# geometrian/simple-spectral

Measured on AMD Instinct MI355X. Metric: Msamples/s (w*h*spp/s) cornell-srgb 512x512, higher is better.
Workload: dtype f32

## Files before the change

include/ssx.h:

```cpp
#ifndef SSX_H
#define SSX_H

#include <stddef.h>
#include <stdint.h>

#ifdef __cplusplus
extern "C" {
#endif

#define SSX_ABI_VERSION 2

enum {
	SSX_OK = 0,
	SSX_ERR_DATA = -1,
	SSX_ERR_ARG = -2,
	SSX_ERR_SCENE = -3,
	SSX_ERR_DEVICE = -10,
	SSX_ERR_STATE = -11
};

#define SSX_MAX_DEPTH 10u
#define SSX_TILE_SIZE 8u
#define SSX_SAMPLE_WAVELENGTHS 4u
#define SSX_MAX_TEXTURES 64u
// ... 232 lines not shown

int ssx_delta_e_images(ssx_ctx* ctx, uint32_t width, uint32_t height, const float* xyz_a, const float* xyz_b, const double white_a[3], const double white_b[3],
                       const uint8_t* labels , uint32_t regions, const double t[2], float* de , float* lab ,
                       double* SUM, double* SSQ, float* MAX, uint64_t* NF, uint64_t* NX, uint64_t* EX );
int ssx_spectral_delta_e(ssx_ctx* ctx, const ssx_denoise_params* denoise , int denoised_a, int denoised_b, const float* weights_a ,
                         const float* weights_b , const double white_a[3], const double white_b[3], const uint8_t* labels , uint32_t regions,
                         const double t[2], float* de , float* lab ,
                         double* SUM, double* SSQ, float* MAX, uint64_t* NF, uint64_t* NX, uint64_t* EX );

enum {
	SSX_DBG_FMATH = 1,
	SSX_DBG_SPHTRI = 2,
	SSX_DBG_ARVO = 3,
	SSX_DBG_SAMPLE_LIGHT = 4,
	SSX_DBG_COSHEMI = 5,
	SSX_DBG_TRACE = 6,
	SSX_DBG_RAND_CHOICE = 7,
	SSX_DBG_ALBEDO = 8,
	SSX_DBG_FLUX_TO_XYZ = 9,
	SSX_DBG_RAND_1F = 10,
	SSX_DBG_GLIBC_MATH = 11,
	SSX_DBG_SPHTRI_GLIBC = 12, SSX_DBG_ARVO_GLIBC = 13, SSX_DBG_SAMPLE_LIGHT_GLIBC = 14, SSX_DBG_COSHEMI_GLIBC = 15,
	SSX_DBG_TRACE_MASKED = 16,
	SSX_DBG_TRACE_TOPO = 17
};
enum {
	SSX_SWEEP_RCP = 1,
	SSX_SWEEP_SQRT = 2,
	SSX_SWEEP_INVERSESQRT = 3,
	SSX_SWEEP_SIN = 4,
	SSX_SWEEP_COS = 5,
	SSX_SWEEP_ACOS = 6,
	SSX_SWEEP_DIV_PI = 7,
	SSX_SWEEP_RCP64 = 8,
	SSX_SWEEP_DIV_PAIRS = 9,
	SSX_SWEEP_ACOS_SIN = 10,
	SSX_SWEEP_SIN_PROOF = 11, SSX_SWEEP_COS_PROOF = 12, SSX_SWEEP_ACOS_PROOF = 13,
	SSX_SWEEP_GLIBC_SIN = 14, SSX_SWEEP_GLIBC_COS = 15, SSX_SWEEP_GLIBC_ACOS = 16,
	SSX_SWEEP_GLIBC_COS_LDS = 17
};
int ssx_debug_sweep(ssx_ctx* ctx, uint32_t op, uint32_t lo, uint64_t count, uint64_t result[11]);
int ssx_debug_pass1_source(const uint8_t* vid, uint32_t n_quads, const char* name, char* out, size_t out_size);
int ssx_debug_eval(ssx_ctx* ctx, uint32_t op, const void* in, uint32_t in_words, void* out, uint32_t out_words, uint32_t n);
int ssx_debug_samples(ssx_ctx* ctx, const ssx_render_params* params, float* xyza, uint64_t* rng_state, uint32_t* levels);
int ssx_debug_sample_flux(ssx_ctx* ctx, const ssx_render_params* params, float* flux, float* lambda_0);
int ssx_debug_tile_mask(ssx_ctx* ctx, const ssx_render_params* params, uint32_t* out);
int ssx_debug_spectral_accumulate(ssx_ctx* ctx, uint32_t width, uint32_t height, uint32_t bins, uint32_t tile_first, uint32_t tile_stride, uint32_t tile_skew,
// ... 62 lines not shown
```

simple_spectral_amd/_capi.py:

```python
import ctypes as C
import os

from . import build as _build


class SsxSpectrum(C.Structure):
    _fields_ = [("offset", C.c_uint32), ("n", C.c_uint32), ("low", C.c_float), ("high", C.c_float),
                ("delta_recip", C.c_float)]


class SsxVertex(C.Structure):
    _fields_ = [("pos", C.c_float * 3), ("st", C.c_float * 2)]


class SsxQuad(C.Structure):
    _fields_ = [("v00", SsxVertex), ("v10", SsxVertex), ("v11", SsxVertex), ("v01", SsxVertex),
                ("normal0", C.c_float * 3), ("normal1", C.c_float * 3),
                ("material", C.c_uint32), ("flags", C.c_uint32)]


class SsxMaterial(C.Structure):
    _fields_ = [("kind", C.c_uint32), ("albedo_mode", C.c_uint32), ("albedo_spectrum", C.c_uint32),
                ("albedo_texture", C.c_uint32), ("emission_spectrum", C.c_uint32)]

# ... 88 lines not shown
               "ssx_spectral_import",
               "ssx_set_spectral_moments", "ssx_spectral_variance", "ssx_spectral_probe", "ssx_probe_arrays",
               "ssx_spectral_noise", "ssx_spectral_noise_reduce",
               "ssx_spectral_moments_import",
               "ssx_spectral_compare", "ssx_spectral_compare_arrays",
               "ssx_delta_e_images", "ssx_spectral_delta_e",
               "ssx_debug_tile_mask", "ssx_debug_spectral_accumulate", "ssx_debug_fold", "ssx_debug_step"]
SSX_FOLD_ROW_WORDS, SSX_FOLD_LAMBDA0, SSX_FOLD_CAM_DIR, SSX_FOLD_HIT, SSX_FOLD_N, SSX_FOLD_LEVEL0, SSX_FOLD_LEVEL_WORDS = 160, 0, 1, 4, 5, 10, 15
SSX_FOLD_L_FS, SSX_FOLD_L_NDL, SSX_FOLD_L_PDF, SSX_FOLD_L_FLAGS, SSX_FOLD_L_EMISSION, SSX_FOLD_L_NEE = 0, 4, 5, 6, 7, 11
SSX_FOLD_EMISSION, SSX_FOLD_NEE, SSX_FOLD_NEE_VISIBLE = 1, 2, 4
SSX_STEP_ROW_WORDS, SSX_STEP_R_ORIG, SSX_STEP_R_DIR, SSX_STEP_R_IGNORE, SSX_STEP_R_DEPTH, SSX_STEP_R_LAMBDA0, SSX_STEP_R_RNG, SSX_STEP_R_PREV_SLOT = 16, 0, 3, 6, 7, 8, 9, 13
SSX_STEP_NO_SLOT, SSX_STEP_OUT_WORDS = 0x1FFF, 40
(SSX_STEP_O_FLAGS, SSX_STEP_O_HIT_TRI, SSX_STEP_O_HIT_DIST, SSX_STEP_O_HIT_ST, SSX_STEP_O_EMISSION, SSX_STEP_O_NEE, SSX_STEP_O_NEE_TERM, SSX_STEP_O_FS, SSX_STEP_O_NDL,
 SSX_STEP_O_PDF, SSX_STEP_O_PREV_SLOT, SSX_STEP_O_TAIL_DEPTH, SSX_STEP_O_TAIL_HIT, SSX_STEP_O_NEXT_ORIG, SSX_STEP_O_NEXT_DIR, SSX_STEP_O_NEXT_IGNORE,
 SSX_STEP_O_NEXT_DEPTH, SSX_STEP_O_RNG, SSX_STEP_O_SLOT) = 0, 1, 2, 3, 5, 9, 13, 17, 21, 22, 23, 24, 25, 26, 29, 32, 33, 34, 36
SSX_STEP_HIT, SSX_STEP_CONTINUED, SSX_STEP_EMISSION, SSX_STEP_PARKED, SSX_STEP_VISIBLE = 1, 2, 4, 8, 16
(SSX_SWEEP_RCP, SSX_SWEEP_SQRT, SSX_SWEEP_INVERSESQRT, SSX_SWEEP_SIN, SSX_SWEEP_COS, SSX_SWEEP_ACOS, SSX_SWEEP_DIV_PI,
 SSX_SWEEP_RCP64, SSX_SWEEP_DIV_PAIRS, SSX_SWEEP_ACOS_SIN, SSX_SWEEP_SIN_PROOF, SSX_SWEEP_COS_PROOF, SSX_SWEEP_ACOS_PROOF) = range(1, 14)
(SSX_DBG_FMATH, SSX_DBG_SPHTRI, SSX_DBG_ARVO, SSX_DBG_SAMPLE_LIGHT, SSX_DBG_COSHEMI, SSX_DBG_TRACE, SSX_DBG_RAND_CHOICE,
 SSX_DBG_ALBEDO, SSX_DBG_FLUX_TO_XYZ, SSX_DBG_RAND_1F) = range(1, 11)
(SSX_DBG_GLIBC_MATH, SSX_DBG_SPHTRI_GLIBC, SSX_DBG_ARVO_GLIBC, SSX_DBG_SAMPLE_LIGHT_GLIBC, SSX_DBG_COSHEMI_GLIBC) = range(11, 16)
(SSX_SWEEP_GLIBC_SIN, SSX_SWEEP_GLIBC_COS, SSX_SWEEP_GLIBC_ACOS, SSX_SWEEP_GLIBC_COS_LDS) = range(14, 18)
SSX_DBG_TRACE_TOPO = 17
SSX_DBG_TRACE_MASKED = 16
HOST_SYMBOLS = ["ssh_scene_create", "ssh_scene_create_ex", "ssh_scene_destroy", "ssh_scene_desc", "ssh_xyza_to_srgba", "ssh_save_image",
                "ssh_load_png_rgb8", "ssh_free", "ssh_color_values", "ssh_last_error", "ssh_checkpoint_save", "ssh_checkpoint_load", "ssh_sums_merge", "ssh_save_npy_f32",
                "ssh_develop_weights", "ssh_relight_gain", "ssh_emitter_spectrum",
                "ssh_checkpoint_save_spectral", "ssh_checkpoint_load_spectral", "ssh_spectral_merge",
                "ssh_probe_derive", "ssh_probe_save_csv", "ssh_spectral_noise_derive", "ssh_spectral_noise_save_csv",
                "ssh_checkpoint_save_moments", "ssh_checkpoint_load_moments", "ssh_moments_merge",
                "ssh_compare_derive", "ssh_compare_save_csv",
                "ssh_delta_e_derive", "ssh_delta_e_save_csv", "ssh_develop_white"]

_hip = None
_host = None


def host_lib():
    global _host
    if _host is None:
        path = _build.HOST_LIB
        if not os.path.exists(path):
            _build.build_host()
        lib = C.CDLL(path)
        vp = C.c_void_p
        lib.ssh_last_error.restype = C.c_char_p
# ... 230 lines not shown
```

simple_spectral_amd/csrc/ssx_api.hip:

```cpp
#include "ssx_kernels.hip"
#include "ssx_debug.hip"

#include "../../include/ssx.h"

#include <chrono>
#include <array>
#include <atomic>
#include <cstdarg>
#include <cstdio>
#include <cstdlib>
#include <cmath>
#include <algorithm>
#include <cstring>
#include <mutex>
#include <string>
#include <thread>
#include <vector>

#include <limits.h>
#include <set>

#include "ssx_jit.h"

namespace {
// ... 1066 lines not shown
	SSX_HIP(ctx, hipMemcpy(d_in.ptr, in, (size_t)n * in_words * 4, hipMemcpyHostToDevice));
	SsxKernelArgs a{};
	a.blob = ctx->d_blob.as<uint32_t>(); a.blob_words = ctx->blob_words; a.rgb_mode = ctx->rgb_mode ? 1u : 0u;
	const size_t lds = staged_blob_lds(ctx->blob_words);
	if (op == SSX_DBG_TRACE_MASKED && in_words < 11u) return fail(ctx, SSX_ERR_ARG, "SSX_DBG_TRACE_MASKED: a row is orig[3], dir[3], ignore, mask[4]");
	if (op == SSX_DBG_TRACE_TOPO) {
		if (in_words < 8u) return fail(ctx, SSX_ERR_ARG, "SSX_DBG_TRACE_TOPO: a row is orig[3], dir[3], ignore, has_ray");
		if (ctx->topology == 0u) return fail(ctx, SSX_ERR_STATE, "SSX_DBG_TRACE_TOPO: the context runs the generic trace (topology 0); that is SSX_DBG_TRACE");
		const uint32_t* d_rows = d_in.as<uint32_t>(); uint32_t* d_res = d_out.as<uint32_t>();
		void* args[] = { &a, &d_rows, &in_words, &d_res, &out_words, &n };
		if (ctx->topology == 3u) {
			std::string err;
			const ssx_jit::Kernels* k = ssx_jit::get(ctx->device, ctx->jit_vid, &err, ssx_jit::kVariantDebug);
			if (!k || !k->debug_trace) return fail(ctx, SSX_ERR_STATE, "SSX_DBG_TRACE_TOPO: the debug kernel of the scene's pattern could not be compiled: " + err);
			SSX_HIP(ctx, hipModuleLaunchKernel(k->debug_trace, (n + 255u) / 256u, 1, 1, 256, 1, 1, (unsigned)lds, ctx->stream, args, nullptr));
		} else {
			const void* host = ctx->topology == 1u ? (const void*)ssx_debug_trace_cornell_kernel : (const void*)ssx_debug_trace_plane_kernel;
			SSX_HIP(ctx, hipLaunchKernel(host, dim3((n + 255u) / 256u), dim3(256), args, lds, ctx->stream));
		}
		SSX_HIP(ctx, hipStreamSynchronize(ctx->stream));
		SSX_HIP(ctx, hipMemcpy(out, d_out.ptr, (size_t)n * out_words * 4, hipMemcpyDeviceToHost));
		return SSX_OK;
	}
	const auto kernel =op >= SSX_DBG_GLIBC_MATH && op <= SSX_DBG_COSHEMI_GLIBC ? ssx_debug_eval_glibc_kernel : ssx_debug_eval_kernel;
	hipLaunchKernelGGL(kernel, dim3((n + 255u) / 256u), dim3(256), lds, ctx->stream, a, op, d_in.as<uint32_t>(), in_words, d_out.as<uint32_t>(), out_words, n);
	SSX_HIP(ctx, hipGetLastError());
	SSX_HIP(ctx, hipStreamSynchronize(ctx->stream));
	SSX_HIP(ctx, hipMemcpy(out, d_out.ptr, (size_t)n * out_words * 4, hipMemcpyDeviceToHost));
	return SSX_OK;
}

int ssx_debug_sweep(ssx_ctx* ctx, uint32_t op, uint32_t lo, uint64_t count, uint64_t result[11]) {
	if (!ctx || !result || count == 0 || count > (1ull << 32)) return SSX_ERR_ARG;
	if (!ctx->have_scene) return fail(ctx, SSX_ERR_STATE, "no scene uploaded");
	if (ctx->rendering.load()) return fail(ctx, SSX_ERR_STATE, "render in progress");
	SSX_HIP(ctx, hipSetDevice(ctx->device));
	DeviceBuffer d_res;
	SSX_HIP(ctx, d_res.reserve(11 * sizeof(unsigned long long)));
	SSX_HIP(ctx, hipMemsetAsync(d_res.ptr, 0, 11 * sizeof(unsigned long long), ctx->stream));
	SsxKernelArgs a{};
	a.blob = ctx->d_blob.as<uint32_t>(); a.blob_words = ctx->blob_words;
	const size_t lds = staged_blob_lds(ctx->blob_words);
	const auto kernel = op >= SSX_SWEEP_GLIBC_SIN ? ssx_debug_sweep_glibc_kernel : ssx_debug_sweep_kernel;
	hipLaunchKernelGGL(kernel, dim3(256 * 16), dim3(256), lds, ctx->stream, a, op, lo, (uint64_t)count, d_res.as<unsigned long long>());
	SSX_HIP(ctx, hipGetLastError());
	SSX_HIP(ctx, hipStreamSynchronize(ctx->stream));
// ... 334 lines not shown
```

simple_spectral_amd/csrc/ssx_debug.hip:

```cpp
#include "../../include/ssx.h"
#include "ssx_ddmath.h"

namespace {

__device__ __forceinline__ Rng load_rng(const uint32_t* w) {
	Rng r;
	r.state = ((uint64_t)w[1] << 32) | w[0];
	r.inc = ((uint64_t)w[3] << 32) | w[2];
	return r;
}
__device__ __forceinline__ float f(uint32_t u) { return __uint_as_float(u); }
__device__ __forceinline__ uint32_t u(float x) { return __float_as_uint(x); }

}

__device__ __forceinline__ uint32_t sweep_hash(uint32_t h) {
	h ^= h >> 16; h *= 0x7FEB352Du; h ^= h >> 15; h *= 0x846CA68Bu; h ^= h >> 16;
	return h;
}
__device__ __forceinline__ bool same_float(float a, float b) { return __float_as_uint(a) == __float_as_uint(b) || (a != a && b != b); }
extern "C" __global__ void __launch_bounds__(256) ssx_debug_sweep_kernel(SsxKernelArgs a, uint32_t op, uint32_t lo, uint64_t count, unsigned long long* res) {
	Lds L; L.w = stage_lds(a);
	(void)L;
	unsigned long long bad = 0, mx = 0;
// ... 157 lines not shown
		float xyz[3];
		flux_to_xyz(L, fl, f(x[4]), xyz);
		o[0] = u(xyz[0]); o[1] = u(xyz[1]); o[2] = u(xyz[2]);
		break;
	}
	case SSX_DBG_RAND_1F: {
		Rng r = load_rng(x);
		o[0] = u(rand_1f(r)); o[1] = (uint32_t)r.state; o[2] = (uint32_t)(r.state >> 32);
		break;
	}
	default: break;
	}
	if (gid < n)
		for (uint32_t k = 0; k < out_words && k < 12u; ++k) out[(size_t)gid * out_words + k] = o[k];
}

#define SSX_DEBUG_TRACE_TOPO_KERNEL(name, topo) \
	extern "C" __global__ void __launch_bounds__(256) name(SsxKernelArgs a, const uint32_t* in, uint32_t in_words, uint32_t* out, uint32_t out_words, uint32_t n) { \
		debug_trace_rows<topo>(a, in, in_words, out, out_words, n); \
	}
SSX_DEBUG_TRACE_TOPO_KERNEL(ssx_debug_trace_cornell_kernel, 1)
SSX_DEBUG_TRACE_TOPO_KERNEL(ssx_debug_trace_plane_kernel, 2)
#undef SSX_DEBUG_TRACE_TOPO_KERNEL

__device__ __forceinline__ uint32_t fold_rank(uint32_t rc, uint32_t seed) { return (rc * ((seed << 1) | 1u) + (seed >> 8)) & (SSX_COHORT_RECORDS - 1u); }
template <bool NARROW, bool GLIBC, bool FLUX>
__device__ __forceinline__ void debug_fold_body(const SsxKernelArgs& a, const uint32_t* rows, uint32_t n_tiles, uint32_t n_k, uint32_t order_seed, uint32_t parked) {
	static_assert((SSX_COHORT_RECORDS & (SSX_COHORT_RECORDS - 1u)) == 0u, "fold_rank permutes a power of two");
	uint32_t* const lds_words = stage_lds<GLIBC>(a);
	Lds L; L.w = lds_words;
	const uint32_t wave = threadIdx.x >> 6, lane = threadIdx.x & 63u;
	const uint32_t wave_slot = blockIdx.x * 4u + wave;
	if (wave_slot >= n_tiles) return;
	uint32_t* const cnt = lds_words + a.blob_words + wave * SSX_WAVE_COUNTER_WORDS;
	const uint32_t rec_base = wave_slot * n_k * 64u;
	const uint32_t* const tile_rows = rows + (size_t)wave_slot * 64u * n_k * SSX_FOLD_ROW_WORDS;
	LogRef lg; lg.cnt = cnt; lg.wave_base = wave_slot * 2u * a.unit_cohorts;
	for (uint32_t kq = 0; kq < n_k; kq += SSX_COHORT_KS) {
		const uint32_t cohort = kq / SSX_COHORT_KS, ways = min(SSX_COHORT_KS, n_k - kq);
		for (uint32_t s = 0; s < ways; ++s) {
			const uint32_t rc = s * 64u + lane, my_rank = fold_rank(rc, order_seed);
			uint32_t fs0 = 0, ne0 = 0;
			for (uint32_t o = 0; o < ways * 64u; ++o) {
				if (fold_rank(o, order_seed) >= my_rank) continue;
				const uint32_t* y = tile_rows + ((size_t)(o & 63u) * n_k + kq + (o >> 6)) * SSX_FOLD_ROW_WORDS;
				const uint32_t on = min(y[SSX_FOLD_N], SSX_MAX_FRAMES);
// ... 280 lines not shown
```

simple_spectral_amd/csrc/ssx_jit.h:

```cpp
#pragma once
#include <hip/hip_runtime.h>
#include <dlfcn.h>

#include <sys/stat.h>
#include <unistd.h>

#include <algorithm>
#include <array>
#include <chrono>
#include <condition_variable>
#include <cstdint>
#include <cstdio>
#include <cstdlib>
#include <cstring>
#include <deque>
#include <map>
#include <mutex>
#include <set>
#include <string>
#include <thread>
#include <utility>
#include <vector>

#include "ssx_sources_gen.h"
// ... 88 lines not shown
	int (*log_size)(Program, size_t*) = nullptr;
	int (*log)(Program, char*) = nullptr;
	int (*code_size)(Program, size_t*) = nullptr;
	int (*code)(Program, char*) = nullptr;
	int (*destroy)(Program*) = nullptr;
	bool open(std::string* err) {
		if (lib) return true;
		for (const char* name : { "libhiprtc.so.7", "libhiprtc.so", "/opt/rocm/lib/libhiprtc.so" }) if ((lib = dlopen(name, RTLD_NOW | RTLD_LOCAL))) break;
		if (!lib) { const char* why = dlerror(); *err = std::string("hipRTC is not available (") + (why ? why : "dlopen failed") + ")"; return false; }
		bool ok = true;
		auto sym = [&](const char* n) { void* s = dlsym(lib, n); ok = ok && s; return s; };
		create = (decltype(create))sym("hiprtcCreateProgram"); compile = (decltype(compile))sym("hiprtcCompileProgram");
		log_size = (decltype(log_size))sym("hiprtcGetProgramLogSize"); log = (decltype(log))sym("hiprtcGetProgramLog");
		code_size = (decltype(code_size))sym("hiprtcGetCodeSize"); code = (decltype(code))sym("hiprtcGetCode");
		destroy = (decltype(destroy))sym("hiprtcDestroyProgram");
		if (!ok) { *err = "hipRTC lacks an entry point"; dlclose(lib); lib = nullptr; }
		return ok;
	}
};

struct Kernels {
	hipModule_t module = nullptr;
	hipFunction_t path = nullptr, path_nq = nullptr;
	hipFunction_t debug_trace = nullptr;
};

enum class State { Missing, Pending, Ready, Failed };

inline uint64_t fnv64(const void* data, size_t n, uint64_t h = 0xCBF29CE484222325ull) {
	const unsigned char* p = static_cast<const unsigned char*>(data);
	for (size_t i = 0; i < n; ++i) { h ^= p[i]; h *= 0x100000001B3ull; }
	return h;
}

struct Shared {
	std::mutex m;
	std::condition_variable cv;
	std::map<std::string, std::string> code, errors;
	std::set<std::string> queued;
	std::deque<std::pair<std::string, std::pair<VidTable, uint32_t>>> jobs;
	bool worker_running = false;
	std::map<std::pair<int, std::string>, Kernels> modules;
	std::set<std::string> disk_missed;
	std::mutex rtc_mutex;
	Rtc rtc;
	uint64_t compiled = 0, disk_hits = 0;
};
// ... 115 lines not shown
	if (libm_flag(libm)) opts.push_back(libm_flag(libm));
	const int rc = rtc.compile(prog, (int)opts.size(), opts.data());
	if (rc != 0) {
		size_t n = 0; rtc.log_size(prog, &n);
		std::string log(n, '\0'); if (n) rtc.log(prog, &log[0]);
		*err = "hipRTC could not compile the specialised kernels: " + log.substr(0, 600);
		rtc.destroy(&prog);
		return false;
	}
	size_t n = 0; rtc.code_size(prog, &n);
	obj->resize(n); rtc.code(prog, &(*obj)[0]);
	rtc.destroy(&prog);
	return true;
}

inline const Kernels* load_locked(Shared& S, int device, const std::string& key, std::string* err) {
	auto it = S.modules.find({ device, key });
	if (it != S.modules.end()) return &it->second;
	const std::string& obj = S.code[key];
	Kernels k;
	hipError_t e = hipModuleLoadData(&k.module, obj.data());
	if (key.compare(0, 6, "debug|") == 0) {
		if (e == hipSuccess) e = hipModuleGetFunction(&k.debug_trace, k.module, "ssx_debug_trace_jit");
	} else {
		if (e == hipSuccess) e = hipModuleGetFunction(&k.path, k.module, "ssx_render_kernel_jit");
		if (e == hipSuccess) e = hipModuleGetFunction(&k.path_nq, k.module, "ssx_render_kernel_jit_nq");
	}
	if (e != hipSuccess) {
		*err = std::string("loading the specialised kernels failed: ") + hipGetErrorString(e);
		if (k.module) (void)hipModuleUnload(k.module);
		S.errors[key] = *err; S.code.erase(key);
		return nullptr;
	}
	return &(S.modules[{ device, key }] = k);
}

inline State lookup(int device, const VidTable& vids, const Kernels** out, std::string* err, uint32_t libm = 0) {
	Shared& S = shared();
	const std::string key = pattern_key(vids, libm);
	{
		std::lock_guard<std::mutex> g(S.m);
		auto bad = S.errors.find(key);
		if (bad != S.errors.end()) { *err = bad->second; return State::Failed; }
		if (S.code.count(key)) { *out = load_locked(S, device, key, err); return *out ? State::Ready : State::Failed; }
		if (S.queued.count(key)) return State::Pending;
		if (S.disk_missed.count(key)) return State::Missing;
// ... 75 lines not shown
```

simple_spectral_amd/csrc/ssx_kernels.hip:

```cpp
#include <hip/hip_runtime.h>
#ifndef __HIPCC_RTC__
#include <stdint.h>
#endif

#include "ssx_blob.h"
#include "ssx_exact.h"
#include "ssx_lanestat.h"
extern __shared__ __attribute__((aligned(16))) uint32_t ssx_lds[];
#define SSX_FM_TABLE (reinterpret_cast<const double*>(ssx_lds))
#ifdef SSX_JIT_BUILD
#include "ssx_fmath.h"
#else
#include "../../include/ssx_fmath.h"
#endif
#define SSX_GM_TABLE (SSX_FM_TABLE + SSX_FM_I_A11)
#ifdef SSX_JIT_BUILD
#include "ssx_glibc_math.h"
#else
#include "../../include/ssx_glibc_math.h"
#endif
__device__ const double ssx_fm_coeff_values[SSX_FM_N_COEFF] = SSX_FM_COEFF_INIT;
__device__ const double ssx_gm_coeff_values[SSX_GM_N_COEFF] = SSX_GM_COEFF_INIT;
static_assert(2 * SSX_FM_N_COEFF <= SSX_LDS_PREFIX_WORDS, "coefficient table");
static_assert(SSX_FM_I_A11 + SSX_GM_N_COEFF <= SSX_FM_N_COEFF, "glibc coefficients in the arc-cosine slots");
// ... 505 lines not shown
				double Ud = (double)B.y * (double)C.x - (double)B.x * (double)C.y;
				double Vd = (double)C.y * (double)A.x - (double)C.x * (double)A.y;
				double Wd = (double)A.y * (double)B.x - (double)A.x * (double)B.y;
				if ((Ud < 0.0 || Vd < 0.0 || Wd < 0.0) && (Ud > 0.0 || Vd > 0.0 || Wd > 0.0)) continue;
				U = (float)Ud; V = (float)Vd; W = (float)Wd;
			}
			float det = U + V + W;
			if (!(__builtin_fabsf(det) > SSX_EPS)) continue;
			float Az = rs.Sz * A.z, Bz = rs.Sz * B.z, Cz = rs.Sz * C.z;
			float T = U * Az + V * Bz + W * Cz;
			if ((__float_as_uint(det) ^ __float_as_uint(T)) & 0x80000000u) continue;
			float det_recip = ssx_exact::rcp(det);
			float dist = T * det_recip;
			if (dist >= SSX_EPS && dist < hit.dist) {
				hit.tri = (int)(2u * base + bit); hit.dist = dist;
				hit.U = U; hit.V = V; hit.W = W; hit.det_recip = det_recip;
				if (which == 0u) cand &= ~(1ull << (bit + 1u));
			}
		}
		if (tm) SSX_TIME_AFTER(*tm, stat_base == 0 ? 8 : 13, hit.dist);
	}
}

struct SphTri {
	V3 A, B, C;
	float b, cos_c;
	float alpha, cos_alpha, sin_alpha;
	float area;
};

template <bool GLIBC = false>
__device__ __forceinline__ void sphtri_make_general(V3 A, V3 B, V3 C, SphTri& t) {
	auto acos_ = [](float x) { return GLIBC ? ssx_glibc_acosf(x) : ssx_acosf_lds(x); };
	auto sin_ = [](float x) { return GLIBC ? ssx_glibc_sinf(x) : ssx_sinf_lds(x); };
	const float under_pi = __uint_as_float(0x40490FDAu);
	const float nanv = __uint_as_float(0x7FC00000u);
	float cos_a = clamp_glm(dot3(B, C), -1.0f, 1.0f);
	float cos_b = clamp_glm(dot3(A, C), -1.0f, 1.0f);
	float cos_c = clamp_glm(dot3(A, B), -1.0f, 1.0f);
	float a = clamp_glm(acos_(cos_a), 0.0f, under_pi);
	float b = clamp_glm(acos_(cos_b), 0.0f, under_pi);
	float c = clamp_glm(acos_(cos_c), 0.0f, under_pi);
	float sin_a = sin_(a), sin_b = sin_(b), sin_c = sin_(c);
	float numer0 = cos_a - cos_b * cos_c;
	float numer1 = cos_b - cos_c * cos_a;
	float numer2 = cos_c - cos_a * cos_b;
// ... 269 lines not shown
	float bx = hit.U * hit.det_recip, by = hit.V * hit.det_recip, bz = hit.W * hit.det_recip;
	const float* s0 = Q.st[0];
	const float* s1 = which ? Q.st[2] : Q.st[1];
	const float* s2 = which ? Q.st[3] : Q.st[2];
	st_x = (bx * s0[0] + by * s1[0]) + bz * s2[0];
	st_y = (bx * s0[1] + by * s1[1]) + bz * s2[1];
}

template <int TOPO>
__device__ __forceinline__ void debug_trace_rows(const SsxKernelArgs& a, const uint32_t* in, uint32_t in_words, uint32_t* out, uint32_t out_words, uint32_t n) {
	Lds L; L.w = stage_lds(a);
	const uint32_t gid = blockIdx.x * blockDim.x + threadIdx.x;
	const uint32_t item = gid < n ? gid : n - 1u;
	const uint32_t* x = in + (size_t)item * in_words;
	HitInfo h;
	trace<TOPO>(L, mk(__uint_as_float(x[0]), __uint_as_float(x[1]), __uint_as_float(x[2])), mk(__uint_as_float(x[3]), __uint_as_float(x[4]), __uint_as_float(x[5])),
	            (int)x[6], x[7] != 0u, h);
	uint32_t o[5] = { h.tri < 0 ? 0xFFFFFFFFu : (uint32_t)h.tri >> 1, h.tri < 0 ? 0u : (uint32_t)h.tri & 1u, __float_as_uint(h.dist), 0u, 0u };
	if (h.tri >= 0) { float sx, sy; hit_st(L.quad((uint32_t)h.tri >> 1), (uint32_t)h.tri & 1u, h, sx, sy); o[3] = __float_as_uint(sx); o[4] = __float_as_uint(sy); }
	if (gid < n)
		for (uint32_t k = 0; k < out_words && k < 5u; ++k) out[(size_t)gid * out_words + k] = o[k];
}

template <bool NARROW, bool BLACK, bool GLIBC = false>
__device__ __forceinline__ bool path_step(const Lds& L, const ShadowQ& q, const SsxKernelArgs& a, const LogRef& lg, Path& p, bool& pushed, uint32_t& level_word) {
	const SsxBlobHeader& h = L.hdr();
	level_word = level_word_none();
	SSX_STAT(4);
	const uint32_t hq = (uint32_t)p.hit_tri >> 1, which = (uint32_t)p.hit_tri & 1u;
	const SsxBlobQuad& Q = L.quad(hq);
	const SsxBlobQuad& M = Q;
	V3 N = mk(Q.normal[which][0], Q.normal[which][1], Q.normal[which][2]);

	float direct[4] = { 0.0f, 0.0f, 0.0f, 0.0f };
	const bool els = a.no_els == 0u;
	if ((els ? (p.depth == 0u && !a.indirect_only) : true) && M.is_emissive != 0u) {
		SSX_STAT(5);
		Hero em = spectrum_hero(L, M.emission, p.lambda_0, h.lambda_step);
#pragma unroll
		for (int k = 0; k < 4; ++k) direct[k] += em.v[k];
		store_emission(a, lg, p.depth, p.rec_index, direct);
		level_word = level_word_emission(level_word);
	}
	if (p.depth + 1u >= SSX_MAX_DEPTH_) return false;
	const V3 hit_pos = add(p.orig, scl(p.hit_dist, p.dir));
	p.orig = hit_pos;
// ... 70 lines not shown
	}
	if (!cont || (els && p.depth + 2u >= SSX_MAX_DEPTH_)) return false;
	SSX_STAT(12);
	const uint32_t slot = log_append(lg, 0u);
	store_level_entry(a, lg, slot, f_s, n_dot_l, pdf_w_i, p.prev_slot, level_word);
	wave_release(lg.cnt);
	p.prev_slot = slot;
	p.dir = w_i; p.ignore = (int)hq;
	++p.depth;
	return true;
}

template <int TOPO, bool NARROW>
__device__ __forceinline__ void shadow_flush(const Lds& L, const SsxKernelArgs& a, const ShadowQ& q, uint32_t first, uint32_t n, SsxTimer& tm) {
	const uint32_t lane = threadIdx.x & 63u;
	const bool have = lane < n;
	const bool narrow = NARROW;
	float4 e0 = make_float4(0.0f, 0.0f, 0.0f, 0.0f), e1 = make_float4(0.0f, 1.0f, 0.0f, 0.0f), e2 = e0;
	if (have) {
		if (narrow) { const float4* E = q.e + 2u * (first + lane); e0 = E[0]; e1 = E[1]; e2.z = e1.z; e2.w = e1.w; }
		else { const float4* E = q.e + 3u * (first + lane); e0 = E[0]; e1 = E[1]; e2 = E[2]; }
	}
	const uint32_t tag = __float_as_uint(e2.z);
	HitInfo sh;
	trace<TOPO>(L, mk(e0.x, e0.y, e0.z), mk(e0.w, e1.x, e1.y), (int)(tag & 0xFFu), have, sh, 2, nullptr, &tm);
	if (have) {
		const bool visible = sh.tri >= 0 && ((uint32_t)sh.tri >> 1) == (tag >> 8);
		store_shadow_outcome<NARROW>(a, __float_as_uint(e2.w), visible, e1.z, e1.w, e2.x, e2.y);
		wave_release(q.cnt);
	}
}

__device__ __forceinline__ const __attribute__((address_space(4))) SsxKernelArgs& cold_args() {
	auto p = __builtin_amdgcn_kernarg_segment_ptr();
	asm volatile("" : "+s"(p));
	return *(const __attribute__((address_space(4))) SsxKernelArgs*)p;
}
__device__ __forceinline__ double ld_agent(const double* p) { return __hip_atomic_load(p, __ATOMIC_RELAXED, __HIP_MEMORY_SCOPE_AGENT); }
__device__ __forceinline__ void st_agent(double* p, double v) { __hip_atomic_store(p, v, __ATOMIC_RELAXED, __HIP_MEMORY_SCOPE_AGENT); }
__device__ __forceinline__ void add_sample(bool rgb_mode, double acc[4], float x, float y, float z, float alpha) {
	if (rgb_mode) { acc[0] += (double)x; acc[1] += (double)y; acc[2] += (double)z; acc[3] += (double)alpha; }
	else { acc[0] += (double)(x * 0.001f); acc[1] += (double)(y * 0.001f); acc[2] += (double)(z * 0.001f); acc[3] += (double)(alpha * 0.001f); }
}
__device__ __forceinline__ void stage_sample(float4* rec, float x, float y, float z, float alpha) {
	uint64_t* const q = reinterpret_cast<uint64_t*>(rec);
	__hip_atomic_store(q, (uint64_t)__float_as_uint(x) | ((uint64_t)__float_as_uint(y) << 32), __ATOMIC_RELAXED, __HIP_MEMORY_SCOPE_AGENT);
	__hip_atomic_store(q + 1, (uint64_t)__float_as_uint(z) | ((uint64_t)__float_as_uint(alpha) << 32), __ATOMIC_RELAXED, __HIP_MEMORY_SCOPE_AGENT);
}
__device__ __forceinline__ void add_staged_sample(bool rgb_mode, double acc[4], const float4* rec) {
	const uint64_t* const q = reinterpret_cast<const uint64_t*>(rec);
// ... 478 lines not shown
		if (!__any(active) && !cur_valid && !more && !old_pending && sq.count == 0u) break;
	}
#ifdef SSX_REGTIME
	if (lane < (uint32_t)SSX_NTIME) atomicAdd(&g_regtime[lane], tm.acc[lane]);
#endif
}

#ifndef SSX_WAVES_PER_EU
#define SSX_WAVES_PER_EU 4
#endif
#ifndef SSX_JIT_GLIBC
#define SSX_JIT_GLIBC 0
#endif
#ifndef SSX_JIT_FLUX
#define SSX_JIT_FLUX 0
#endif
#define SSX_PATH_KERNEL(name, topo, narrow, glibc, flux) \
	extern "C" __global__ void __launch_bounds__(256) __attribute__((amdgpu_waves_per_eu(SSX_WAVES_PER_EU))) name(SsxKernelArgs a) { render_body<topo, narrow, false, glibc, flux>(a); }
#ifdef SSX_JIT_BUILD
#ifdef SSX_JIT_DEBUG
extern "C" __global__ void __launch_bounds__(256) ssx_debug_trace_jit(SsxKernelArgs a, const uint32_t* in, uint32_t in_words, uint32_t* out, uint32_t out_words, uint32_t n) {
	debug_trace_rows<3>(a, in, in_words, out, out_words, n);
}
#else
SSX_PATH_KERNEL(ssx_render_kernel_jit, 3, false, SSX_JIT_GLIBC, SSX_JIT_FLUX)
SSX_PATH_KERNEL(ssx_render_kernel_jit_nq, 3, true, SSX_JIT_GLIBC, SSX_JIT_FLUX)
#endif
#else
SSX_PATH_KERNEL(ssx_render_kernel, 0, false, false, false)
SSX_PATH_KERNEL(ssx_render_kernel_cornell, 1, false, false, false)
#ifndef SSX_PROBE_BUILD
SSX_PATH_KERNEL(ssx_render_kernel_plane, 2, false, false, false)
SSX_PATH_KERNEL(ssx_render_kernel_nq, 0, true, false, false)
SSX_PATH_KERNEL(ssx_render_kernel_cornell_nq, 1, true, false, false)
SSX_PATH_KERNEL(ssx_render_kernel_plane_nq, 2, true, false, false)
SSX_PATH_KERNEL(ssx_render_kernel_glibc, 0, false, true, false)
SSX_PATH_KERNEL(ssx_render_kernel_cornell_glibc, 1, false, true, false)
SSX_PATH_KERNEL(ssx_render_kernel_plane_glibc, 2, false, true, false)
SSX_PATH_KERNEL(ssx_render_kernel_nq_glibc, 0, true, true, false)
SSX_PATH_KERNEL(ssx_render_kernel_cornell_nq_glibc, 1, true, true, false)
SSX_PATH_KERNEL(ssx_render_kernel_plane_nq_glibc, 2, true, true, false)
SSX_PATH_KERNEL(ssx_render_kernel_flux, 0, false, false, true)
SSX_PATH_KERNEL(ssx_render_kernel_cornell_flux, 1, false, false, true)
SSX_PATH_KERNEL(ssx_render_kernel_plane_flux, 2, false, false, true)
SSX_PATH_KERNEL(ssx_render_kernel_nq_flux, 0, true, false, true)
SSX_PATH_KERNEL(ssx_render_kernel_cornell_nq_flux, 1, true, false, true)
// ... 40 lines not shown
```

Measured before the change: 3222.

## Add dedicated shadow-ray visibility trace with early exit on light occlusion

Replaces the general closest-hit trace used for shadow rays with a specialized trace_shadow routine. It tests the light quad's triangles first, then considers only occluders that could be nearer, and stops once the light is known to be blocked. The goal is to skip intersection work for triangles that cannot change the visible/occluded verdict. It adds a debug kernel and API op for checking verdicts against the full trace; the risk is extra branching and divergence, plus verdicts that may differ subtly from the reference tie-breaking.

```diff
diff --git a/include/ssx.h b/include/ssx.h
--- a/include/ssx.h
+++ b/include/ssx.h
@@ -278,7 +278,8 @@
 	SSX_DBG_GLIBC_MATH = 11,
 	SSX_DBG_SPHTRI_GLIBC = 12, SSX_DBG_ARVO_GLIBC = 13, SSX_DBG_SAMPLE_LIGHT_GLIBC = 14, SSX_DBG_COSHEMI_GLIBC = 15,
 	SSX_DBG_TRACE_MASKED = 16,
-	SSX_DBG_TRACE_TOPO = 17
+	SSX_DBG_TRACE_TOPO = 17,
+	SSX_DBG_SHADOW_VERDICT = 18
 };
 enum {
 	SSX_SWEEP_RCP = 1,
diff --git a/simple_spectral_amd/_capi.py b/simple_spectral_amd/_capi.py
--- a/simple_spectral_amd/_capi.py
+++ b/simple_spectral_amd/_capi.py
@@ -134,6 +134,7 @@
 (SSX_DBG_GLIBC_MATH, SSX_DBG_SPHTRI_GLIBC, SSX_DBG_ARVO_GLIBC, SSX_DBG_SAMPLE_LIGHT_GLIBC, SSX_DBG_COSHEMI_GLIBC) = range(11, 16)
 (SSX_SWEEP_GLIBC_SIN, SSX_SWEEP_GLIBC_COS, SSX_SWEEP_GLIBC_ACOS, SSX_SWEEP_GLIBC_COS_LDS) = range(14, 18)
 SSX_DBG_TRACE_TOPO = 17
+SSX_DBG_SHADOW_VERDICT = 18
 SSX_DBG_TRACE_MASKED = 16
 HOST_SYMBOLS = ["ssh_scene_create", "ssh_scene_create_ex", "ssh_scene_destroy", "ssh_scene_desc", "ssh_xyza_to_srgba", "ssh_save_image",
                 "ssh_load_png_rgb8", "ssh_free", "ssh_color_values", "ssh_last_error", "ssh_checkpoint_save", "ssh_checkpoint_load", "ssh_sums_merge", "ssh_save_npy_f32",
diff --git a/simple_spectral_amd/csrc/ssx_api.hip b/simple_spectral_amd/csrc/ssx_api.hip
--- a/simple_spectral_amd/csrc/ssx_api.hip
+++ b/simple_spectral_amd/csrc/ssx_api.hip
@@ -1112,6 +1112,23 @@
 		SSX_HIP(ctx, hipMemcpy(out, d_out.ptr, (size_t)n * out_words * 4, hipMemcpyDeviceToHost));
 		return SSX_OK;
 	}
+	if (op == SSX_DBG_SHADOW_VERDICT) {
+		if (in_words < 9u) return fail(ctx, SSX_ERR_ARG, "SSX_DBG_SHADOW_VERDICT: a row is orig[3], dir[3], ignore, light, has_ray");
+		const uint32_t* d_rows = d_in.as<uint32_t>(); uint32_t* d_res = d_out.as<uint32_t>();
+		void* args[] = { &a, &d_rows, &in_words, &d_res, &out_words, &n };
+		if (ctx->topology == 3u) {
+			std::string err;
+			const ssx_jit::Kernels* k = ssx_jit::get(ctx->device, ctx->jit_vid, &err, ssx_jit::kVariantDebug);
+			if (!k || !k->debug_shadow) return fail(ctx, SSX_ERR_STATE, "SSX_DBG_SHADOW_VERDICT: the debug kernel of the scene's pattern could not be compiled: " + err);
+			SSX_HIP(ctx, hipModuleLaunchKernel(k->debug_shadow, (n + 255u) / 256u, 1, 1, 256, 1, 1, (unsigned)lds, ctx->stream, args, nullptr));
+		} else {
+			const void* host = ctx->topology == 1u ? (const void*)ssx_debug_shadow_cornell_kernel : ctx->topology == 2u ? (const void*)ssx_debug_shadow_plane_kernel : (const void*)ssx_debug_shadow_kernel;
+			SSX_HIP(ctx, hipLaunchKernel(host, dim3((n + 255u) / 256u), dim3(256), args, lds, ctx->stream));
+		}
+		SSX_HIP(ctx, hipStreamSynchronize(ctx->stream));
+		SSX_HIP(ctx, hipMemcpy(out, d_out.ptr, (size_t)n * out_words * 4, hipMemcpyDeviceToHost));
+		return SSX_OK;
+	}
 	const auto kernel =op >= SSX_DBG_GLIBC_MATH && op <= SSX_DBG_COSHEMI_GLIBC ? ssx_debug_eval_glibc_kernel : ssx_debug_eval_kernel;
 	hipLaunchKernelGGL(kernel, dim3((n + 255u) / 256u), dim3(256), lds, ctx->stream, a, op, d_in.as<uint32_t>(), in_words, d_out.as<uint32_t>(), out_words, n);
 	SSX_HIP(ctx, hipGetLastError());
diff --git a/simple_spectral_amd/csrc/ssx_debug.hip b/simple_spectral_amd/csrc/ssx_debug.hip
--- a/simple_spectral_amd/csrc/ssx_debug.hip
+++ b/simple_spectral_amd/csrc/ssx_debug.hip
@@ -203,6 +203,15 @@
 SSX_DEBUG_TRACE_TOPO_KERNEL(ssx_debug_trace_cornell_kernel, 1)
 SSX_DEBUG_TRACE_TOPO_KERNEL(ssx_debug_trace_plane_kernel, 2)
 #undef SSX_DEBUG_TRACE_TOPO_KERNEL
+
+#define SSX_DEBUG_SHADOW_KERNEL(name, topo) \
+	extern "C" __global__ void __launch_bounds__(256) name(SsxKernelArgs a, const uint32_t* in, uint32_t in_words, uint32_t* out, uint32_t out_words, uint32_t n) { \
+		debug_shadow_rows<topo>(a, in, in_words, out, out_words, n); \
+	}
+SSX_DEBUG_SHADOW_KERNEL(ssx_debug_shadow_kernel, 0)
+SSX_DEBUG_SHADOW_KERNEL(ssx_debug_shadow_cornell_kernel, 1)
+SSX_DEBUG_SHADOW_KERNEL(ssx_debug_shadow_plane_kernel, 2)
+#undef SSX_DEBUG_SHADOW_KERNEL
 
 __device__ __forceinline__ uint32_t fold_rank(uint32_t rc, uint32_t seed) { return (rc * ((seed << 1) | 1u) + (seed >> 8)) & (SSX_COHORT_RECORDS - 1u); }
 template <bool NARROW, bool GLIBC, bool FLUX>
diff --git a/simple_spectral_amd/csrc/ssx_jit.h b/simple_spectral_amd/csrc/ssx_jit.h
--- a/simple_spectral_amd/csrc/ssx_jit.h
+++ b/simple_spectral_amd/csrc/ssx_jit.h
@@ -134,7 +134,7 @@
 struct Kernels {
 	hipModule_t module = nullptr;
 	hipFunction_t path = nullptr, path_nq = nullptr;
-	hipFunction_t debug_trace = nullptr;
+	hipFunction_t debug_trace = nullptr, debug_shadow = nullptr;
 };
 
 enum class State { Missing, Pending, Ready, Failed };
@@ -296,6 +296,7 @@
 	hipError_t e = hipModuleLoadData(&k.module, obj.data());
 	if (key.compare(0, 6, "debug|") == 0) {
 		if (e == hipSuccess) e = hipModuleGetFunction(&k.debug_trace, k.module, "ssx_debug_trace_jit");
+		if (e == hipSuccess) e = hipModuleGetFunction(&k.debug_shadow, k.module, "ssx_debug_shadow_jit");
 	} else {
 		if (e == hipSuccess) e = hipModuleGetFunction(&k.path, k.module, "ssx_render_kernel_jit");
 		if (e == hipSuccess) e = hipModuleGetFunction(&k.path_nq, k.module, "ssx_render_kernel_jit_nq");
diff --git a/simple_spectral_amd/csrc/ssx_kernels.hip b/simple_spectral_amd/csrc/ssx_kernels.hip
--- a/simple_spectral_amd/csrc/ssx_kernels.hip
+++ b/simple_spectral_amd/csrc/ssx_kernels.hip
@@ -551,6 +551,123 @@
 	}
 }
 
+template <int TOPO>
+__device__ __forceinline__ float shadow_tri_dist(const Lds& L, const RaySetup& rs, bool perm_hbm, const float* gperm, uint32_t bit) {
+	const uint32_t q = bit >> 1, which = bit & 1u;
+	float pv3[9];
+	if constexpr (TOPO != 0) {
+		struct alignas(16) V3a { float x, y, z; };
+		const uint2 to = L.triofs(bit);
+		const char* vt = L.vtab4(rs.perm);
+		const V3a A3 = *reinterpret_cast<const V3a*>(vt + (to.x & 0xFFFFu)), B3 = *reinterpret_cast<const V3a*>(vt + (to.x >> 16)), C3 = *reinterpret_cast<const V3a*>(vt + to.y);
+		pv3[0] = A3.x; pv3[1] = A3.y; pv3[2] = A3.z; pv3[3] = B3.x; pv3[4] = B3.y; pv3[5] = B3.z; pv3[6] = C3.x; pv3[7] = C3.y; pv3[8] = C3.z;
+	} else {
+		float2 Axy, Bxy, Cxy; float Az_, Bz_, Cz_;
+		if (perm_hbm) {
+			const float* pq = gperm + q * SSX_PERM_WORDS_PER_QUAD + rs.perm * 12u;
+			Axy = *reinterpret_cast<const float2*>(pq); Bxy = *reinterpret_cast<const float2*>(pq + 2u + 2u * which); Cxy = *reinterpret_cast<const float2*>(pq + 4u + 2u * which);
+			Az_ = pq[8]; Bz_ = pq[9u + which]; Cz_ = pq[10u + which];
+		} else {
+			const float* lq = L.perm(q, rs.perm);
+			Axy = *reinterpret_cast<const float2*>(lq); Bxy = *reinterpret_cast<const float2*>(lq + 2u + 2u * which); Cxy = *reinterpret_cast<const float2*>(lq + 4u + 2u * which);
+			Az_ = lq[8]; Bz_ = lq[9u + which]; Cz_ = lq[10u + which];
+		}
+		pv3[0] = Axy.x; pv3[1] = Axy.y; pv3[2] = Az_; pv3[3] = Bxy.x; pv3[4] = Bxy.y; pv3[5] = Bz_; pv3[6] = Cxy.x; pv3[7] = Cxy.y; pv3[8] = Cz_;
+	}
+	const float never = __builtin_inff();
+	SV A = shear_xyz(pv3[0], pv3[1], pv3[2], rs), B = shear_xyz(pv3[3], pv3[4], pv3[5], rs), C = shear_xyz(pv3[6], pv3[7], pv3[8], rs);
+	float U = B.y * C.x - B.x * C.y;
+	float V = C.y * A.x - C.x * A.y;
+	float W = A.y * B.x - A.x * B.y;
+	if (__builtin_fminf(__builtin_fminf(__builtin_fabsf(U), __builtin_fabsf(V)), __builtin_fabsf(W)) == 0.0f) {
+		double Ud = (double)B.y * (double)C.x - (double)B.x * (double)C.y;
+		double Vd = (double)C.y * (double)A.x - (double)C.x * (double)A.y;
+		double Wd = (double)A.y * (double)B.x - (double)A.x * (double)B.y;
+		if ((Ud < 0.0 || Vd < 0.0 || Wd < 0.0) && (Ud > 0.0 || Vd > 0.0 || Wd > 0.0)) return never;
+		U = (float)Ud; V = (float)Vd; W = (float)Wd;
+	}
+	float det = U + V + W;
+	if (!(__builtin_fabsf(det) > SSX_EPS)) return never;
+	float Az = rs.Sz * A.z, Bz = rs.Sz * B.z, Cz = rs.Sz * C.z;
+	float T = U * Az + V * Bz + W * Cz;
+	if ((__float_as_uint(det) ^ __float_as_uint(T)) & 0x80000000u) return never;
+	float dist = T * ssx_exact::rcp(det);
+	return dist >= SSX_EPS ? dist : never;
+}
+
+template <int TOPO>
+__device__ __forceinline__ bool trace_shadow(const Lds& L, V3 orig, V3 dir, int ignore_quad, uint32_t light_quad, bool has_ray, SsxTimer* tm = nullptr) {
+	const SsxBlobHeader& hd = L.hdr();
+	const uint32_t nq = hd.n_quads;
+	if (TOPO == 0 && nq > 32u) {
+		HitInfo sh;
+		trace<TOPO>(L, orig, dir, ignore_quad, has_ray, sh, 2, nullptr, tm);
+		return sh.tri >= 0 && ((uint32_t)sh.tri >> 1) == light_quad;
+	}
+	const RaySetup rs = ray_setup(orig, dir);
+	SSX_STAT(2);
+	const bool perm_hbm = TOPO == 0 && hd.perm_hbm != 0u;
+	const float* const gperm = reinterpret_cast<const float*>(((uint64_t)hd.perm_ptr_hi << 32) | (uint64_t)hd.perm_ptr_lo);
+	auto quad_flags = [&](const float* perm_of_quad, uint32_t& acc) {
+		float pv[12];
+		load_perm(perm_of_quad, pv);
+		SV a = shear_vertex(pv, 0, rs), b = shear_vertex(pv, 1, rs), c = shear_vertex(pv, 2, rs), d = shear_vertex(pv, 3, rs);
+		float U0 = b.y * c.x - b.x * c.y;
+		float V0 = c.y * a.x - c.x * a.y;
+		float W0 = a.y * b.x - a.x * b.y;
+		float U1 = c.y * d.x - c.x * d.y;
+		float V1 = d.y * a.x - d.x * a.y;
+		float W1 = -V0;
+		float mn0 = __builtin_fminf(__builtin_fminf(U0, V0), W0), mx0 = __builtin_fmaxf(__builtin_fmaxf(U0, V0), W0);
+		float mn1 = __builtin_fminf(__builtin_fminf(U1, V1), W1), mx1 = __builtin_fmaxf(__builtin_fmaxf(U1, V1), W1);
+		acc = __builtin_amdgcn_alignbit(acc, __float_as_uint(__builtin_fmaf(mn0, mx0, 0.0f)), 31u);
+		acc = __builtin_amdgcn_alignbit(acc, __float_as_uint(__builtin_fmaf(mn1, mx1, 0.0f)), 31u);
+	};
+	uint32_t acc0 = 0u, acc1 = 0u;
+	const uint32_t n0 = min(nq, 16u), n1 = nq - n0;
+	if constexpr (TOPO == 1) pass1_cornell(L.vtab(rs.perm), rs, acc0, acc1);
+	else if constexpr (TOPO == 2) pass1_plane(L.vtab(rs.perm), rs, acc0, acc1);
+#ifdef SSX_JIT_BUILD
+	else if constexpr (TOPO == 3) pass1_jit(L.vtab(rs.perm), rs, acc0, acc1);
+#endif
+	else if (!perm_hbm) {
+		for (uint32_t q = 0; q < n0; ++q) quad_flags(L.perm(q, rs.perm), acc0);
+		for (uint32_t q = 16u; q < nq; ++q) quad_flags(L.perm(q, rs.perm), acc1);
+	} else {
+		for (uint32_t q = 0; q < n0; ++q) quad_flags(gperm + q * SSX_PERM_WORDS_PER_QUAD + rs.perm * 12u, acc0);
+		for (uint32_t q = 16u; q < nq; ++q) quad_flags(gperm + q * SSX_PERM_WORDS_PER_QUAD + rs.perm * 12u, acc1);
+	}
+	const uint32_t mixed0 = __builtin_bitreverse32(acc0) >> (32u - 2u * n0);
+	const uint32_t mixed1 = n1 ? __builtin_bitreverse32(acc1) >> (32u - 2u * n1) : 0u;
+	const uint64_t valid = TOPO == 0 ? hd.tri_valid[0] : (nq >= 32u ? ~0ull : ((1ull << (2u * nq)) - 1ull));
+	uint64_t cand = ~(((uint64_t)mixed1 << 32) | (uint64_t)mixed0) & valid;
+	const uint32_t ign = (uint32_t)ignore_quad;
+	if (ign < 32u) cand &= ~(3ull << (2u * ign));
+	if (!has_ray) cand = 0ull;
+	if (tm) SSX_TIME_AFTER(*tm, 12, (uint32_t)cand ^ (uint32_t)(cand >> 32));
+	const uint32_t lsh = 2u * (light_quad & 31u);
+	uint32_t lc = light_quad < 32u ? (uint32_t)(cand >> lsh) & 3u : 0u;
+	cand &= ~(3ull << lsh);
+	bool visible = lc != 0u;
+	if (!visible) cand = 0ull;
+	float d0L = __builtin_inff(), d1L = __builtin_inff(), r = __builtin_inff();
+	while (lc != 0u || cand != 0ull) {
+		SSX_STAT(3);
+		const bool of_light = lc != 0u;
+		const uint32_t bit = of_light ? lsh + (uint32_t)__builtin_ctz(lc) : (uint32_t)__builtin_ctzll(cand);
+		if (of_light) lc &= lc - 1u; else cand &= cand - 1ull;
+		const uint32_t q = bit >> 1, which = bit & 1u;
+		const float d = shadow_tri_dist<TOPO>(L, rs, perm_hbm, gperm, bit);
+		if (of_light) { if (which == 0u) d0L = d; else d1L = d; }
+		else if (q < light_quad && d < r) { r = d; if (which == 0u) cand &= ~(1ull << (bit + 1u)); }
+		const float dL = d0L < r ? d0L : d1L;
+		const bool lost = !(dL < r) || (q > light_quad && d < dL);
+		if (lost && lc == 0u) { visible = false; cand = 0ull; }
+	}
+	if (tm) SSX_TIME_AFTER(*tm, 13, (uint32_t)visible);
+	return visible;
+}
+
 struct SphTri {
 	V3 A, B, C;
 	float b, cos_c;
@@ -866,6 +983,21 @@
 		for (uint32_t k = 0; k < out_words && k < 5u; ++k) out[(size_t)gid * out_words + k] = o[k];
 }
 
+template <int TOPO>
+__device__ __forceinline__ void debug_shadow_rows(const SsxKernelArgs& a, const uint32_t* in, uint32_t in_words, uint32_t* out, uint32_t out_words, uint32_t n) {
+	Lds L; L.w = stage_lds(a);
+	const uint32_t gid = blockIdx.x * blockDim.x + threadIdx.x;
+	uint32_t x[9] = { 0u, 0u, 0u, 0u, 0x3F800000u, 0u, 0u, 0u, 0u };
+	if (gid < n)
+		for (uint32_t k = 0; k < 9u; ++k) x[k] = in[(size_t)gid * in_words + k];
+	const bool visible = trace_shadow<TOPO>(L, mk(__uint_as_float(x[0]), __uint_as_float(x[1]), __uint_as_float(x[2])), mk(__uint_as_float(x[3]), __uint_as_float(x[4]), __uint_as_float(x[5])),
+	                                        (int)x[6], x[7], gid < n && x[8] != 0u);
+	if (gid < n) {
+		out[(size_t)gid * out_words] = visible ? 1u : 0u;
+		for (uint32_t k = 1; k < out_words; ++k) out[(size_t)gid * out_words + k] = 0u;
+	}
+}
+
 template <bool NARROW, bool BLACK, bool GLIBC = false>
 __device__ __forceinline__ bool path_step(const Lds& L, const ShadowQ& q, const SsxKernelArgs& a, const LogRef& lg, Path& p, bool& pushed, uint32_t& level_word) {
 	const SsxBlobHeader& h = L.hdr();
@@ -982,10 +1114,8 @@
 		else { const float4* E = q.e + 3u * (first + lane); e0 = E[0]; e1 = E[1]; e2 = E[2]; }
 	}
 	const uint32_t tag = __float_as_uint(e2.z);
-	HitInfo sh;
-	trace<TOPO>(L, mk(e0.x, e0.y, e0.z), mk(e0.w, e1.x, e1.y), (int)(tag & 0xFFu), have, sh, 2, nullptr, &tm);
+	const bool visible = trace_shadow<TOPO>(L, mk(e0.x, e0.y, e0.z), mk(e0.w, e1.x, e1.y), (int)(tag & 0xFFu), tag >> 8, have, &tm);
 	if (have) {
-		const bool visible = sh.tri >= 0 && ((uint32_t)sh.tri >> 1) == (tag >> 8);
 		store_shadow_outcome<NARROW>(a, __float_as_uint(e2.w), visible, e1.z, e1.w, e2.x, e2.y);
 		wave_release(q.cnt);
 	}
@@ -1510,6 +1640,9 @@
 extern "C" __global__ void __launch_bounds__(256) ssx_debug_trace_jit(SsxKernelArgs a, const uint32_t* in, uint32_t in_words, uint32_t* out, uint32_t out_words, uint32_t n) {
 	debug_trace_rows<3>(a, in, in_words, out, out_words, n);
 }
+extern "C" __global__ void __launch_bounds__(256) ssx_debug_shadow_jit(SsxKernelArgs a, const uint32_t* in, uint32_t in_words, uint32_t* out, uint32_t out_words, uint32_t n) {
+	debug_shadow_rows<3>(a, in, in_words, out, out_words, n);
+}
 #else
 SSX_PATH_KERNEL(ssx_render_kernel_jit, 3, false, SSX_JIT_GLIBC, SSX_JIT_FLUX)
 SSX_PATH_KERNEL(ssx_render_kernel_jit_nq, 3, true, SSX_JIT_GLIBC, SSX_JIT_FLUX)
```

Result: no change. 3230, median of 6 (+0.3%).
